# MakisChristou/fhestring

Measured on AMD Instinct MI355X. Metric: PBS/sec and ms/op for contains() on N-char FheString, higher is better.
Workload: dtype f64

## Files before the change

### __graft_entry__.py

```python
import os
import subprocess
import sys

ROOT = os.path.dirname(os.path.abspath(__file__))
if ROOT not in sys.path:
    sys.path.insert(0, ROOT)


def build():
    subprocess.check_call(["make", "-s", "-j4", "-C", os.path.join(ROOT, "fhestring_amd", "csrc")])
    subprocess.check_call(["make", "-s", "-C", os.path.join(ROOT, "oracle"), "liboracle.so"])
    subprocess.check_call(["gcc", "-std=c99", "-Wall", "-Wextra", "-pedantic", "-Werror", "-I", os.path.join(ROOT, "include"),
                           os.path.join(ROOT, "examples", "c_host.c"), "-L", os.path.join(ROOT, "fhestring_amd"),
                           "-lfhestring_hip", "-Wl,-rpath,$ORIGIN/../fhestring_amd", "-o", os.path.join(ROOT, "examples", "c_host")])
    import fhestring_amd
    fhestring_amd.lib()
    from oracle import core
    core.lib()


def smoke():
    import numpy as np
    import fhestring_amd
    from fhestring_amd.api import MyServerKey
# ... 2 lines not shown
    osk = core.ServerKey(keys)
    sk = MyServerKey.from_raw_keys(keys.bsk, keys.ksk, arith=fhestring_amd.Context.ARITH_F64_FFT)
    names = ["msg", "eq_biv", "sign"]
    luts = np.stack([radix.lut_poly(n) for n in names])
    cts = np.stack([keys.encrypt_block(m) for m in (0, 3, 9, 15, 22, 31)])
    idx = np.array([0, 1, 2, 0, 2, 1], np.uint32)
    got = sk.ctx.pbs_batch(cts, idx, luts)
    assert np.array_equal(got, osk.pbs_batch(cts, idx, luts, mode=3)), "HIP FFT PBS differs from the CPU mirror"
    sk.ctx.set_arithmetic(sk.ctx.ARITH_EXACT_NTT)
    got = sk.ctx.pbs_batch(cts, idx, luts)
    assert np.array_equal(got, osk.pbs_batch(cts, idx, luts)), "HIP PBS differs from the CPU oracle"
    osk.set_mb2(keys.bsk_mb2)
    sk.ctx.set_arithmetic(sk.ctx.ARITH_F64_FFT)
    sk.ctx.load_multibit_key(keys.bsk_mb2)
    sk.ctx.set_arithmetic(sk.ctx.ARITH_F64_FFT_MB2)
    got = sk.ctx.pbs_batch(cts, idx, luts)
    assert np.array_equal(got, osk.pbs_batch(cts, idx, luts, mode=4)), "HIP two-bit PBS differs from the CPU mirror"
    sk.ctx.set_arithmetic(sk.ctx.ARITH_EXACT_NTT)
    sk.ctx.load_multibit_key(keys.bsk_mb2)
    sk.ctx.set_arithmetic(sk.ctx.ARITH_EXACT_NTT_MB2)
    got = sk.ctx.pbs_batch(cts, idx, luts)
    assert np.array_equal(got, osk.pbs_batch(cts, idx, luts, mode=5)), "HIP exact two-bit PBS differs from the CPU oracle"
    sk.ctx.set_arithmetic(sk.ctx.ARITH_EXACT_NTT)
    sk.set_mode(1)
    s = sk.upload_string(np.stack([keys.encrypt_char(b) for b in b"zama!\0"]))
    res = sk.contains_clear(s, "ma")
    assert keys.decrypt_char(res.download()) == 1
    res = sk.contains_clear(s, "xy")
    assert keys.decrypt_char(res.download()) == 0
    sk.close()
    _smoke_rekey()
    print("smoke ok: PBS bit-exact vs oracle (exact NTT, f64 FFT, both with two key bits per product too), "
          "contains() decrypts correctly, store re-key equals the host reference and decrypts under the new key, "
          "find / rfind / len / flag counts beyond 255 decrypt correctly")


def _smoke_rekey():
    import numpy as np
    from fhestring_amd import FhsError
    from fhestring_amd.api import CompactFheString, MyClientKey, MyServerKey, rekey_host
    N = 2048
    chosen = (0x00000000, 0x00008000, 0x7FFF8000, 0x80000000, 0xFFFFFFFF, 0x00007FFF)
    a, b = MyClientKey(0x5EEDA), MyClientKey(0x5EEDB)
    sk = MyServerKey.from_client_key(a)
    sk.load_packing_key(a)
    key = a.rekey_key(b)
    sk.load_rekey_key(key)
    rng = np.random.default_rng(3)

    def words(n_blocks):
        g = (n_blocks + N - 1) // N
        mask = rng.integers(0, 1 << 32, (g, N), dtype=np.uint32)
        if g == len(chosen):
            mask[:] = np.array(chosen, np.uint32)[:, None]
        return mask, rng.integers(0, 1 << 32, n_blocks, dtype=np.uint32)
# ... 86 lines not shown
```

### bindings/fhestring_hip.rs

```rust
#![allow(non_camel_case_types, dead_code)]
use std::os::raw::{c_char, c_int, c_void};

pub const FHS_LWE_N: c_int = 742;
pub const FHS_POLY_N: c_int = 2048;
pub const FHS_BIG_CT: c_int = 2049;
pub const FHS_SMALL_CT: c_int = 743;
pub const FHS_BLOCKS_PER_CHAR: c_int = 4;
pub const FHS_CHAR_WORDS: usize = 8196;
pub const FHS_BSK_WORDS: usize = 6078464;
pub const FHS_KSK_WORDS: usize = 7608320;
pub const FHS_MAX_FIND_LENGTH: c_int = 255;
pub const FHS_MAX_REPETITIONS: c_int = 16;
pub const FHS_MAX_FIND_LENGTH_WIDE: c_int = 65535;
pub const FHS_WIDE_ABSENT: c_int = 65535;
pub const FHS_OK: c_int = 0;
pub const FHS_ERR_ARG: c_int = -1;
pub const FHS_ERR_HIP: c_int = -2;
pub const FHS_ERR_STATE: c_int = -3;
pub const FHS_ERR_LIMIT: c_int = -4;
pub const FHS_ARITH_EXACT_NTT: c_int = 0;
pub const FHS_ARITH_F64_FFT: c_int = 1;
pub const FHS_ARITH_F64_FFT_MB2: c_int = 2;
pub const FHS_ARITH_EXACT_NTT_MB2: c_int = 3;
pub const FHS_BSK_MB2_WORDS: usize = 9117696;
// ... 62 lines not shown
    pub pbs_shared: u64,
    pub pbs_extracted: u64,
}

#[link(name = "fhestring_hip")]
extern "C" {
    pub fn fhs_ctx_create(device_id: c_int, out: *mut *mut fhs_ctx) -> c_int;
    pub fn fhs_ctx_create_planner(out: *mut *mut fhs_ctx) -> c_int;
    pub fn fhs_ctx_destroy(ctx: *mut fhs_ctx);
    pub fn fhs_last_error(ctx: *const fhs_ctx) -> *const c_char;
    pub fn fhs_load_server_key(ctx: *mut fhs_ctx, bsk: *const u64, ksk: *const u64) -> c_int;
    pub fn fhs_load_multibit_key(ctx: *mut fhs_ctx, bsk_mb2: *const u64) -> c_int;
    pub fn fhs_set_arithmetic(ctx: *mut fhs_ctx, arith: c_int) -> c_int;
    pub fn fhs_get_arithmetic(ctx: *const fhs_ctx) -> c_int;
    pub fn fhs_set_fft4_max_batch(ctx: *mut fhs_ctx, max_batch: c_int) -> c_int;
    pub fn fhs_set_launch_chunk(ctx: *mut fhs_ctx, arith: c_int, n_ciphertexts: usize) -> c_int;
    pub fn fhs_fft_tables(w_re: *mut f64, w_im: *mut f64, u_re: *mut f64, u_im: *mut f64);
    pub fn fhs_fft_mono_table(mono: *mut f64);
    pub fn fhs_pbs_batch(ctx: *mut fhs_ctx, r#in: *const u64, lut_idx: *const u32, luts: *const u64, n_luts: usize, out: *mut u64, B: usize) -> c_int;
    pub fn fhs_keyswitch_modswitch_batch(ctx: *mut fhs_ctx, r#in: *const u64, ms_out: *mut u32, B: usize) -> c_int;
    pub fn fhs_pbs_batch_shifted(ctx: *mut fhs_ctx, r#in: *const u64, lut_idx: *const u32, luts: *const u64, n_luts: usize, shifts: *const u32, n_shifts: usize, out: *mut u64, B: usize) -> c_int;
    pub fn fhs_set_rotation_sharing(ctx: *mut fhs_ctx, on: c_int) -> c_int;
    pub fn fhs_debug_blind_rotate_batch(ctx: *mut fhs_ctx, ks: *const u64, lut_idx: *const u32, luts: *const u64, n_luts: usize, out: *mut u64, B: usize) -> c_int;
    pub fn fhs_pbs_batch_device(ctx: *mut fhs_ctx, d_in: *const u64, d_lut_idx: *const u32, d_luts: *const u64, d_out: *mut u64, B: usize, hip_stream: *mut c_void) -> c_int;
    pub fn fhs_kernel_timing(ctx: *mut fhs_ctx, reset: c_int, blind_rotate_ms: *mut f64, keyswitch_ms: *mut f64, n_blind_rotate: *mut u64, n_keyswitch: *mut u64, pbs_in_launches: *mut u64) -> c_int;
    pub fn fhs_kernel_timing_kind(ctx: *mut fhs_ctx, kind: c_int, avg_ms: *mut f64, launches: *mut u64, pbs_in_launches: *mut u64) -> c_int;
    pub fn fhs_trivial(ctx: *mut fhs_ctx, value: u8) -> fhs_char_t;
    pub fn fhs_upload(ctx: *mut fhs_ctx, blocks: *const u64) -> fhs_char_t;
    pub fn fhs_upload_string(ctx: *mut fhs_ctx, blocks: *const u64, n: usize, out: *mut fhs_char_t) -> c_int;
    pub fn fhs_eq(ctx: *mut fhs_ctx, a: fhs_char_t, b: fhs_char_t) -> fhs_char_t;
    pub fn fhs_ne(ctx: *mut fhs_ctx, a: fhs_char_t, b: fhs_char_t) -> fhs_char_t;
    pub fn fhs_le(ctx: *mut fhs_ctx, a: fhs_char_t, b: fhs_char_t) -> fhs_char_t;
    pub fn fhs_lt(ctx: *mut fhs_ctx, a: fhs_char_t, b: fhs_char_t) -> fhs_char_t;
    pub fn fhs_ge(ctx: *mut fhs_ctx, a: fhs_char_t, b: fhs_char_t) -> fhs_char_t;
    pub fn fhs_gt(ctx: *mut fhs_ctx, a: fhs_char_t, b: fhs_char_t) -> fhs_char_t;
    pub fn fhs_bitand(ctx: *mut fhs_ctx, a: fhs_char_t, b: fhs_char_t) -> fhs_char_t;
    pub fn fhs_bitor(ctx: *mut fhs_ctx, a: fhs_char_t, b: fhs_char_t) -> fhs_char_t;
    pub fn fhs_sub(ctx: *mut fhs_ctx, a: fhs_char_t, b: fhs_char_t) -> fhs_char_t;
    pub fn fhs_add(ctx: *mut fhs_ctx, a: fhs_char_t, b: fhs_char_t) -> fhs_char_t;
    pub fn fhs_if_then_else(ctx: *mut fhs_ctx, cond: fhs_char_t, t: fhs_char_t, f: fhs_char_t) -> fhs_char_t;
    pub fn fhs_flip(ctx: *mut fhs_ctx, a: fhs_char_t) -> fhs_char_t;
    pub fn fhs_is_whitespace(ctx: *mut fhs_ctx, a: fhs_char_t) -> fhs_char_t;
    pub fn fhs_is_uppercase(ctx: *mut fhs_ctx, a: fhs_char_t) -> fhs_char_t;
    pub fn fhs_is_lowercase(ctx: *mut fhs_ctx, a: fhs_char_t) -> fhs_char_t;
    pub fn fhs_clone(ctx: *mut fhs_ctx, a: fhs_char_t) -> fhs_char_t;
    pub fn fhs_release(ctx: *mut fhs_ctx, a: fhs_char_t) -> c_int;
// ... 161 lines not shown
```

### fhestring_amd/api.py

```python
import ctypes as C

import numpy as np

from . import cabi
from ._lib import FhsError, lib, check_single_hip_runtime

_K = dict(cabi.parse_header()["consts"])
BIG_CT = _K["FHS_BIG_CT"]
SMALL_CT = _K["FHS_SMALL_CT"]
POLY_N = _K["FHS_POLY_N"]
PACK_GROUP = _K["FHS_PACK_GROUP"]
PACK_KEY_WORDS = _K["FHS_PACK_KEY_WORDS"]
REKEY_KEY_WORDS = _K["FHS_REKEY_KEY_WORDS"]


def _ptr(a):
    return a.ctypes.data_as(C.c_void_p)


class Context:

    def __init__(self, device_id=0, planner=False):
        self._L = lib()
        if not planner:
# ... 111 lines not shown
                                          _ptr(out), B))
        return out

    def pbs_batch_shifted(self, cts, lut_idx, luts, shifts):
        cts = np.ascontiguousarray(cts, np.uint64).reshape(-1, BIG_CT)
        luts = np.ascontiguousarray(luts, np.uint64).reshape(-1, POLY_N)
        lut_idx = np.ascontiguousarray(lut_idx, np.uint32)
        B = cts.shape[0]
        shifts = np.ascontiguousarray(shifts, np.uint32).reshape(B, -1)
        out = np.zeros((B, shifts.shape[1], BIG_CT), np.uint64)
        self._check(self._L.fhs_pbs_batch_shifted(self._h, _ptr(cts), _ptr(lut_idx), _ptr(luts), luts.shape[0],
                                                  _ptr(shifts), shifts.shape[1], _ptr(out), B))
        return out

    def set_rotation_sharing(self, on=True):
        self._check(self._L.fhs_set_rotation_sharing(self._h, int(bool(on))))

    def keyswitch_modswitch_batch(self, cts):
        cts = np.ascontiguousarray(cts, np.uint64).reshape(-1, BIG_CT)
        B = cts.shape[0]
        out = np.zeros((B, SMALL_CT), np.uint32)
        self._check(self._L.fhs_keyswitch_modswitch_batch(self._h, _ptr(cts), _ptr(out), B))
        return out

    def pbs_batch_device(self, d_in, d_lut_idx, d_luts, d_out, B, stream=0):
        self._check(self._L.fhs_pbs_batch_device(self._h, C.c_void_p(d_in), C.c_void_p(d_lut_idx),
                                                 C.c_void_p(d_luts), C.c_void_p(d_out), int(B),
                                                 C.c_void_p(stream)))

    def kernel_timing(self, reset=False):
        br, ks = C.c_double(), C.c_double()
        nb, nk, units = C.c_uint64(), C.c_uint64(), C.c_uint64()
        narrow = self.kernel_timing_kind(2)
        self._check(self._L.fhs_kernel_timing(self._h, int(reset), C.byref(br), C.byref(ks), C.byref(nb),
                                              C.byref(nk), C.byref(units)))
        return {"blind_rotate_ms": br.value, "keyswitch_ms": ks.value, "n_blind_rotate": nb.value,
                "n_keyswitch": nk.value, "pbs_in_launches": units.value,
                "fft4_ms": narrow[0], "n_fft4": narrow[1], "pbs_in_fft4": narrow[2]}

    def kernel_timing_kind(self, kind):
        ms, n, u = C.c_double(), C.c_uint64(), C.c_uint64()
        self._check(self._L.fhs_kernel_timing_kind(self._h, int(kind), C.byref(ms), C.byref(n), C.byref(u)))
        return ms.value, n.value, u.value


CHAR_WORDS = _K["FHS_CHAR_WORDS"]
# ... 1122 lines not shown
```

### fhestring_amd/csrc/capi_core.cpp

```cpp
#include <algorithm>
#include <new>

#include "capi_internal.h"
#include "keyfile.h"
#include "luts.h"
#include "seeded_kernels.h"

extern "C" {

int fhs_ctx_create(int device_id, fhs_ctx **out) {
    if (!out) return FHS_ERR_ARG;
    *out = nullptr;
    fhs_ctx *c = new (std::nothrow) fhs_ctx();
    if (!c) return FHS_ERR_STATE;
    int rc = c->eng.ctx.init(device_id);
    if (rc) {
        *out = c;
        return rc;
    }
    *out = c;
    return FHS_OK;
}

int fhs_ctx_create_planner(fhs_ctx **out) {
// ... 109 lines not shown
    return e == hipSuccess ? FHS_OK : c.hip_fail(e, "device keystream");
}

int fhs_pbs_batch(fhs_ctx *ctx, const uint64_t *in, const uint32_t *lut_idx, const uint64_t *luts,
                  size_t n_luts, uint64_t *out, size_t B) {
    if (!ctx) return FHS_ERR_ARG;
    return ctx->eng.ctx.pbs_batch_host(in, lut_idx, luts, n_luts, out, B);
}

int fhs_pbs_batch_shifted(fhs_ctx *ctx, const uint64_t *in, const uint32_t *lut_idx, const uint64_t *luts, size_t n_luts,
                          const uint32_t *shifts, size_t n_shifts, uint64_t *out, size_t B) {
    if (!ctx) return FHS_ERR_ARG;
    if (ctx->eng.planner) return ctx->eng.ctx.fail(FHS_ERR_STATE, "planner context: nothing is computed");
    return ctx->eng.ctx.pbs_batch_shifted_host(in, lut_idx, luts, n_luts, shifts, n_shifts, out, B);
}

int fhs_debug_blind_rotate_batch(fhs_ctx *ctx, const uint64_t *ks, const uint32_t *lut_idx, const uint64_t *luts,
                                 size_t n_luts, uint64_t *out, size_t B) {
    if (!ctx) return FHS_ERR_ARG;
    if (ctx->eng.planner) return ctx->eng.ctx.fail(FHS_ERR_STATE, "planner context: nothing is computed");
    return ctx->eng.ctx.blind_rotate_host(ks, lut_idx, luts, n_luts, out, B);
}

int fhs_keyswitch_modswitch_batch(fhs_ctx *ctx, const uint64_t *in, uint32_t *ms_out, size_t B) {
    if (!ctx) return FHS_ERR_ARG;
    return ctx->eng.ctx.ks_ms_batch_host(in, ms_out, B);
}

int fhs_pbs_batch_device(fhs_ctx *ctx, const uint64_t *d_in, const uint32_t *d_lut_idx, const uint64_t *d_luts,
                         uint64_t *d_out, size_t B, void *hip_stream) {
    if (!ctx) return FHS_ERR_ARG;
    if (!d_in || !d_lut_idx || !d_luts || !d_out) return ctx->eng.ctx.fail(FHS_ERR_ARG, "null device pointer");
    return ctx->eng.ctx.pbs_batch_device(d_in, d_lut_idx, d_luts, d_out, B,
                                         hip_stream ? (hipStream_t)hip_stream : ctx->eng.ctx.stream);
}

int fhs_debug_capture_pbs_inputs(fhs_ctx *ctx, size_t max_rows_per_level) {
    if (!ctx) return FHS_ERR_ARG;
    if (int rc = ctx->eng.flush()) return rc;
    ctx->eng.capture_max_rows = max_rows_per_level;
    if (!max_rows_per_level) {
        ctx->eng.capture_rows.clear(); ctx->eng.capture_rows.shrink_to_fit();
        ctx->eng.capture_recs.clear();
    }
    return FHS_OK;
}
// ... 95 lines not shown
```

### fhestring_amd/csrc/context.cpp

```cpp
#include "context.h"
#include "pack_kernels.h"
#include "rekey_kernels.h"
#include "seeded_kernels.h"
#include "../../include/fhestring_hip.h"

#include <algorithm>
#include <cstdlib>
#include <utility>

namespace fhs {

namespace {
constexpr size_t KSK_BYTES = (size_t)BIG_N * KS_LEVEL * SMALL_CT * sizeof(uint64_t);
constexpr size_t BSK_BYTES = (size_t)LWE_N * 4 * POLY_N * sizeof(uint64_t);
}

#define HIP_TRY(expr, what)                                \
    do {                                                   \
        hipError_t e__ = (expr);                           \
        if (e__ != hipSuccess) return hip_fail(e__, what); \
    } while (0)

Event KernelTimer::get() {
    if (pool.empty()) return Event();
// ... 179 lines not shown
        for (int k = 0; k < 3; k++) ok = ok && ur[k] == ht.u_re[k] && ui[k] == ht.u_im[k];
        if (!ok) return fail(-3, "fft_consts.inc does not match the libm-derived twiddles (regenerate it)");
    }
    std::vector<double> flat;
    auto put = [&](const std::vector<double> &v) {
        const size_t at = flat.size();
        flat.insert(flat.end(), v.begin(), v.end());
        return at;
    };
    const size_t at_lanetab = put(ht.lanetab), at_weff = put(ht.weff), at_mono = put(ht.mono), at_r16 = put(ht.r16);
    HIP_TRY(d_fft_tables.reserve_exact(flat.size() * sizeof(double)), "hipMalloc fft tables");
    HIP_TRY(hipMemcpy(d_fft_tables.ptr, flat.data(), flat.size() * sizeof(double), hipMemcpyHostToDevice), "copy fft tables");
    const double *const tab = d_fft_tables.as<double>();
    ft.lanetab = tab + at_lanetab; ft.weff = tab + at_weff; ft.mono = tab + at_mono; ft.r16 = tab + at_r16;
    const size_t n = (size_t)LWE_N * 4 * POLY_N;
    HIP_TRY(d_bsk_fft.reserve_exact(n * sizeof(double)), "hipMalloc bsk fft");
    hipError_t e = launch_bsk_to_fft(d_bsk_std.as<uint64_t>(), d_bsk_fft.as<double>(), ft.lanetab, stream);
    if (e == hipSuccess) e = hipStreamSynchronize(stream);
    if (e != hipSuccess) d_bsk_fft.release();
    HIP_TRY(e, "bsk -> Fourier domain");
    return 0;
}

int Context::keyswitch(const uint64_t *d_in, size_t B, hipStream_t s) {
    if (dig_buf.cap < ks_digits_bytes((int)B)) {
        HIP_TRY(hipStreamSynchronize(s), "sync");
        HIP_TRY(dig_buf.reserve(ks_digits_bytes((int)B)), "hipMalloc digits");
    }
    timer.begin(1, B, s);
    hipError_t e = launch_keyswitch_mfma(d_in, d_ksk_planes.as<int8_t>(), dig_buf.as<int8_t>(), ks_buf.as<uint64_t>(), (int)B, s,
                                         wg_slots / 4);
    timer.end(s);
    if (e != hipSuccess) return hip_fail(e, "keyswitch launch");
    return 0;
}

int Context::set_arithmetic(int mode) {
    if (mode < 0 || mode >= N_ARITH) return fail(-1, "unknown arithmetic mode");
    if (is_f64_fft(mode) && key_loaded && !d_bsk_fft)
        if (int rc = build_fft_key()) return rc;
    if (mode == FHS_ARITH_F64_FFT_MB2 && key_loaded && !d_bsk_mb)
        return fail(-3, "the two-bits-per-product arithmetic needs the pair key in the Fourier domain: call "
                        "fhs_load_multibit_key while arithmetic 1 (f64 FFT) is selected, then fhs_set_arithmetic 2");
    if (mode == FHS_ARITH_EXACT_NTT_MB2 && key_loaded && !d_bsk_ntt_mb)
        return fail(-3, "the exact two-bits-per-product arithmetic needs the pair key converted to residues: call "
                        "fhs_load_multibit_key while the EXACT arithmetic (fhs_set_arithmetic 0) is selected, then "
                        "fhs_set_arithmetic 3");
    arith = mode;
    return 0;
}

int Context::load_multibit_key(const uint64_t *bsk_mb2) {
    if (!bsk_mb2) return fail(-1, "null key pointer");
    if (!key_loaded) return fail(-3, "load the server key before the pair key");
    HIP_TRY(hipSetDevice(device), "hipSetDevice");
    if (!is_f64_fft(arith)) {
// ... 208 lines not shown
                              out_buf.as<uint64_t>(), nullptr, B, stream))
        return rc;
    HIP_TRY(hipMemcpyAsync(out, out_buf.ptr, B * BIG_CT * 8, hipMemcpyDeviceToHost, stream), "D2H");
    HIP_TRY(hipStreamSynchronize(stream), "sync");
    return 0;
}

int Context::ks_ms_batch_host(const uint64_t *in, uint32_t *ms_out, size_t B) {
    if (!key_loaded) return fail(-3, "server key not loaded");
    if (!in || !ms_out) return fail(-1, "null pointer");
    if (B == 0) return 0;
    HIP_TRY(hipSetDevice(device), "hipSetDevice");
    HIP_TRY(in_buf.reserve(B * BIG_CT * 8), "hipMalloc");
    HIP_TRY(ms_buf.reserve(B * SMALL_CT * 4), "hipMalloc");
    HIP_TRY(ks_buf.reserve(B * SMALL_CT * 8), "hipMalloc");
    HIP_TRY(hipMemcpyAsync(in_buf.ptr, in, B * BIG_CT * 8, hipMemcpyHostToDevice, stream), "H2D");
    if (int rc = keyswitch(in_buf.as<uint64_t>(), B, stream)) return rc;
    HIP_TRY(launch_modswitch(ks_buf.as<uint64_t>(), ms_buf.as<uint32_t>(), (int)B, stream), "modswitch launch");
    HIP_TRY(hipMemcpyAsync(ms_out, ms_buf.ptr, B * SMALL_CT * 4, hipMemcpyDeviceToHost, stream), "D2H");
    HIP_TRY(hipStreamSynchronize(stream), "sync");
    return 0;
}

}
```

### fhestring_amd/csrc/context.h

```cpp
#pragma once
#include <hip/hip_runtime.h>

#include <cstdint>
#include <string>
#include <vector>

#include "../../include/fhestring_hip.h"
#include "dist.h"
#include "fft_tables.h"
#include "hip_owners.h"
#include "ntt_tables.h"
#include "pbs_kernels.h"

namespace fhs {

constexpr int N_ARITH = 4;
constexpr bool is_f64_fft(int arith) { return arith == FHS_ARITH_F64_FFT || arith == FHS_ARITH_F64_FFT_MB2; }

struct FftTablePtrs {
    const double *lanetab = nullptr;
    const double *weff = nullptr;
    const double *mono = nullptr;
    const double *r16 = nullptr;
};
// ... 25 lines not shown
    DevBuf d_tables;
    NttTables tw{};
    double crt_c = 0;

    int arith = FHS_ARITH_EXACT_NTT;
    DevBuf d_bsk_fft;
    DevBuf d_bsk_std;
    DevBuf d_fft_tables;
    FftTablePtrs ft;
    DevBuf d_work_counter;
    int wg_slots = 1024;
    DevBuf d_bsk_mb;
    DevBuf d_bsk_ntt_mb;
    const double *d_ntt_mono = nullptr;
    DevBuf d_pack_key_ntt;
    int load_packing_key(const uint64_t *key);
    DevBuf d_rekey_key_ntt;
    int load_rekey_key(const uint64_t *key);
    int load_multibit_key(const uint64_t *bsk_mb2);
    int fft4_max_batch = 512;
    size_t launch_chunk[N_ARITH] = {};
    int set_arithmetic(int mode);
    int keyswitch(const uint64_t *d_in, size_t B, hipStream_t s);
    int blind_rotate(const uint64_t *d_ks, const uint32_t *d_lut_idx, const uint64_t *d_luts, uint64_t *d_out,
                     uint64_t *const *d_out_ptrs, size_t B, hipStream_t s, uint64_t *const *d_body_ptrs = nullptr);

    Dist dist;
    DevBuf xchg_send, xchg_recv;

    DevBuf dig_buf;
    DevBuf ks_buf, ms_buf, in_buf, out_buf, lutidx_buf, luts_buf, tab_buf;
    DevBuf pack_ws[2], pack_tab, pack_out;
    KernelTimer timer;

    int init(int device_id);
    ~Context();
    int fail(int code, const std::string &msg) { err = msg; return code; }
    int hip_fail(hipError_t e, const char *what);

    int load_server_key(const uint64_t *bsk, const uint64_t *ksk);
    int load_compressed_server_key(const uint32_t seed[8], const uint64_t *bsk_bodies, const uint64_t *ksk_bodies);
    int install_server_key(const uint64_t *bsk, const uint64_t *d_ksk);
    int build_fft_key();
    int pbs_batch_device(const uint64_t *d_in, const uint32_t *d_lut_idx, const uint64_t *d_luts,
                         uint64_t *d_out, size_t B, hipStream_t s);
    int pbs_batch_shifted_host(const uint64_t *in, const uint32_t *lut_idx, const uint64_t *luts, size_t n_luts,
                               const uint32_t *shifts, size_t S, uint64_t *out, size_t B);
    int pbs_batch_host(const uint64_t *in, const uint32_t *lut_idx, const uint64_t *luts, size_t n_luts,
                       uint64_t *out, size_t B);
    int ks_ms_batch_host(const uint64_t *in, uint32_t *ms_out, size_t B);
    int blind_rotate_host(const uint64_t *ks, const uint32_t *lut_idx, const uint64_t *luts, size_t n_luts,
                          uint64_t *out, size_t B);
};

}
```

### fhestring_amd/csrc/engine.cpp

```cpp
#include "engine.h"
#include "../../include/fhestring_hip.h"

#include <algorithm>
#include <cstdio>
#include <cstdlib>
#include <cstring>
#include <map>

namespace fhs {

int Engine::on_key_loaded() {
    if (!d_luts_) {
        std::vector<uint64_t> host((size_t)LUT_COUNT * POLY_N);
        for (int id = 0; id < LUT_COUNT; id++) make_lut_poly(id, host.data() + (size_t)id * POLY_N);
        hipError_t e = d_luts_.reserve_exact(host.size() * 8);
        if (e != hipSuccess) return ctx.hip_fail(e, "hipMalloc luts");
        e = hipMemcpy(d_luts_.ptr, host.data(), host.size() * 8, hipMemcpyHostToDevice);
        if (e != hipSuccess) return ctx.hip_fail(e, "copy luts");
    }
    return 0;
}

Engine::~Engine() {
    if (!planner && ctx.stream) (void)hipStreamSynchronize(ctx.stream);
// ... 706 lines not shown
    const size_t stride = (cnt + capture_max_rows - 1) / capture_max_rows;
    for (size_t i = 0; i < cnt; i += stride) {
        const size_t at = capture_rows.size();
        capture_rows.resize(at + BIG_CT);
        hipError_t e = hipMemcpyAsync(capture_rows.data() + at, batch_in_.as<uint64_t>() + (batch_row + i) * BIG_CT, BIG_CT * 8,
                                      hipMemcpyDeviceToHost, ctx.stream);
        if (e == hipSuccess) e = hipStreamSynchronize(ctx.stream);
        if (e != hipSuccess) return ctx.hip_fail(e, "capture download");
        CaptureRec r = l.recs[first + i];
        r.level = level;
        capture_recs.push_back(r);
    }
    return 0;
}

int Engine::launch_rows(const GroupView &v, size_t lo, size_t cnt, uint64_t *dense_out, const TickLevel *levels,
                        size_t n_levels, size_t first_level) {
    const uint8_t *dp = tick_buf_.as<uint8_t>();
    const LinDesc *d_desc = reinterpret_cast<const LinDesc *>(dp);
    const LinTerm *d_terms = reinterpret_cast<const LinTerm *>(dp + v.off_terms);
    const uint32_t *d_lut = reinterpret_cast<const uint32_t *>(dp + v.off_lut);
    uint64_t *const *d_out = reinterpret_cast<uint64_t *const *>(dp + v.off_out);
    uint64_t *const *d_body = reinterpret_cast<uint64_t *const *>(dp + v.off_body);
    hipError_t e = launch_lincomb(d_desc + lo, d_terms, batch_in_.as<uint64_t>(), (int)cnt, ctx.stream);
    if (e != hipSuccess) return ctx.hip_fail(e, "lincomb launch");
    size_t row0 = 0;
    for (size_t j = 0; j < n_levels && capture_max_rows; j++) {
        const TickLevel &l = levels[j];
        const size_t w = l.descs.size(), a = std::max(lo, row0), b = std::min(lo + cnt, row0 + w);
        if (l.recs.size() == w && a < b)
            if (int rc = sample_capture(l, a - row0, b - a, a - lo, (uint32_t)(first_level + j))) return rc;
        row0 += w;
    }
    if (int rc = ctx.keyswitch(batch_in_.as<uint64_t>(), cnt, ctx.stream)) return rc;
    return ctx.blind_rotate(ctx.ks_buf.as<uint64_t>(), d_lut + lo, d_luts_.as<uint64_t>(), dense_out, dense_out ? nullptr : d_out + lo, cnt,
                            ctx.stream, v.n_ext && !dense_out ? d_body + lo : nullptr);
}

int Engine::scatter_rows(const uint64_t *d_all, uint64_t *const *d_out, size_t width) {
    hipError_t e = launch_scatter_blocks(d_all, d_out, (int)width, ctx.stream);
    return e == hipSuccess ? 0 : ctx.hip_fail(e, "scatter launch");
}

void Engine::trace_group(const std::vector<TickLevel> &levels, size_t width) {
    for (auto &l : levels) {
        for (size_t k = 0; k < l.descs.size(); k++) {
            const LinDesc &d = l.descs[k];
            trace_.insert(trace_.end(), {TR_ROW, (uint64_t)(uintptr_t)l.out[k], l.lut[k], d.konst_body >> DELTA_LOG, d.n_terms});
            for (uint32_t t = 0; t < d.n_terms; t++) {
                trace_.push_back((uint64_t)(uintptr_t)l.terms[d.first_term + t].src);
                trace_.push_back((uint64_t)l.terms[d.first_term + t].coef);
            }
        }
        for (const ShareRow &f : l.ext)
            trace_.insert(trace_.end(), {TR_EXT, (uint64_t)(uintptr_t)l.out[f.lead_row], (uint64_t)(uintptr_t)f.out, f.K});
    }
    trace_.push_back(TR_GROUP_END);
// ... 169 lines not shown
```

### fhestring_amd/csrc/pbs_kernels.h

```cpp
#pragma once
#include <hip/hip_runtime.h>
#include <cstddef>
#include <cstdint>

namespace fhs {

constexpr int LWE_N = 742;
constexpr int POLY_N = 2048;
constexpr int BIG_N = 2048;
constexpr int BIG_CT = 2049;
constexpr int SMALL_CT = 743;
constexpr int KS_LEVEL = 5;
constexpr int KS_BASE_LOG = 3;
constexpr int DELTA_LOG = 59;
constexpr int BSK_QUANT_BITS = 6;

constexpr uint64_t NTT_P0 = 140737488273409ull;
constexpr uint64_t NTT_P1 = 140737488252929ull;
constexpr uint64_t NTT_PSI0 = 124135596386681ull;
constexpr uint64_t NTT_PSI1 = 116052249937262ull;

struct NttTables {
    const double *fwd_uni;
    const double *fwd_lane;
// ... 71 lines not shown

size_t blind_rotate_lds_bytes();
hipError_t prepare_device_for_kernels();
hipError_t read_device_ntt_consts(double *fwd_uni , double *inv_uni , double *crt);
hipError_t launch_blind_rotate(const BlindRotateParams &p, hipStream_t s);
hipError_t launch_blind_rotate_fft(const BlindRotateFftParams &p, hipStream_t s);
hipError_t launch_blind_rotate_fft4(const BlindRotateFftParams &p, hipStream_t s);
hipError_t launch_bsk_to_fft(const uint64_t *d_bsk_std, double *d_out, const double *d_lanetab, hipStream_t s,
                             int n_polys = LWE_N * 4);
hipError_t launch_blind_rotate_mb2(const BlindRotateMb2Params &p, hipStream_t s);
hipError_t launch_blind_rotate_ntt_mb2(const BlindRotateNttMb2Params &p, hipStream_t s);
hipError_t prepare_device_for_ntt_mb2();
hipError_t prepare_device_for_fft4();
hipError_t prepare_device_for_keyswitch();
void fft_uniform_consts(double *w_re, double *w_im, double *u_re, double *u_im);
size_t ks_planes_bytes();
size_t ks_digits_bytes(int B);
hipError_t launch_ksk_to_planes(const uint64_t *d_ksk, int8_t *d_planes, hipStream_t s);
hipError_t launch_keyswitch_mfma(const uint64_t *d_in , const int8_t *d_planes, int8_t *d_dig ,
                                 uint64_t *d_ks_out , int B, hipStream_t s, int n_cus = 256);
hipError_t launch_modswitch(const uint64_t *d_ks, uint32_t *d_ms , int B, hipStream_t s);
hipError_t launch_lincomb(const LinDesc *d_desc, const LinTerm *d_terms, uint64_t *d_out ,
                          int n, hipStream_t s);
hipError_t launch_scatter_blocks(const uint64_t *d_in, uint64_t *const *d_dst, int n, hipStream_t s);
hipError_t launch_gather_rows(const uint64_t *const *d_src, uint64_t *d_out, int n, hipStream_t s);
struct ExtractDesc {
    const uint64_t *lead;
    const uint64_t *body;
    uint64_t *out;
    uint32_t K, pad;
};
hipError_t launch_extract_shift(const ExtractDesc *d_desc, int n, hipStream_t s);

}
```

### include/fhestring_hip.h

```cpp
#ifndef FHESTRING_HIP_H
#define FHESTRING_HIP_H

#include <stddef.h>
#include <stdint.h>

#ifdef __cplusplus
extern "C" {
#endif

#define FHS_LWE_N 742
#define FHS_POLY_N 2048
#define FHS_BIG_CT 2049
#define FHS_SMALL_CT 743
#define FHS_BLOCKS_PER_CHAR 4
#define FHS_CHAR_WORDS (4 * 2049)
#define FHS_BSK_WORDS ((size_t)742 * 4 * 2048)
#define FHS_KSK_WORDS ((size_t)2048 * 5 * 743)
#define FHS_MAX_FIND_LENGTH 255
#define FHS_MAX_REPETITIONS 16
#define FHS_MAX_FIND_LENGTH_WIDE 65535
#define FHS_WIDE_ABSENT 65535

#define FHS_OK 0
#define FHS_ERR_ARG (-1)
// ... 11 lines not shown
const char *fhs_last_error(const fhs_ctx *ctx);
int fhs_load_server_key(fhs_ctx *ctx, const uint64_t *bsk, const uint64_t *ksk);
#define FHS_ARITH_EXACT_NTT 0
#define FHS_ARITH_F64_FFT 1
#define FHS_ARITH_F64_FFT_MB2 2
#define FHS_ARITH_EXACT_NTT_MB2 3
#define FHS_BSK_MB2_WORDS ((size_t)371 * 3 * 4 * 2048)
int fhs_load_multibit_key(fhs_ctx *ctx, const uint64_t *bsk_mb2 );
int fhs_set_arithmetic(fhs_ctx *ctx, int arith);
int fhs_get_arithmetic(const fhs_ctx *ctx);
int fhs_set_fft4_max_batch(fhs_ctx *ctx, int max_batch);
int fhs_set_launch_chunk(fhs_ctx *ctx, int arith, size_t n_ciphertexts);
void fhs_fft_tables(double *w_re, double *w_im, double *u_re, double *u_im);
void fhs_fft_mono_table(double *mono );

int fhs_pbs_batch(fhs_ctx *ctx, const uint64_t *in, const uint32_t *lut_idx, const uint64_t *luts,
                  size_t n_luts, uint64_t *out, size_t B);
int fhs_keyswitch_modswitch_batch(fhs_ctx *ctx, const uint64_t *in, uint32_t *ms_out, size_t B);
int fhs_pbs_batch_shifted(fhs_ctx *ctx, const uint64_t *in, const uint32_t *lut_idx, const uint64_t *luts, size_t n_luts,
                          const uint32_t *shifts , size_t n_shifts, uint64_t *out, size_t B);
int fhs_set_rotation_sharing(fhs_ctx *ctx, int on);
int fhs_debug_blind_rotate_batch(fhs_ctx *ctx, const uint64_t *ks, const uint32_t *lut_idx, const uint64_t *luts,
                                 size_t n_luts, uint64_t *out, size_t B);
int fhs_pbs_batch_device(fhs_ctx *ctx, const uint64_t *d_in, const uint32_t *d_lut_idx,
                         const uint64_t *d_luts, uint64_t *d_out, size_t B, void *hip_stream);
int fhs_kernel_timing(fhs_ctx *ctx, int reset, double *blind_rotate_ms, double *keyswitch_ms,
                      uint64_t *n_blind_rotate, uint64_t *n_keyswitch, uint64_t *pbs_in_launches);
int fhs_kernel_timing_kind(fhs_ctx *ctx, int kind, double *avg_ms, uint64_t *launches, uint64_t *pbs_in_launches);

fhs_char_t fhs_trivial(fhs_ctx *ctx, uint8_t value);
fhs_char_t fhs_upload(fhs_ctx *ctx, const uint64_t *blocks );
int fhs_upload_string(fhs_ctx *ctx, const uint64_t *blocks, size_t n, fhs_char_t *out);
fhs_char_t fhs_eq(fhs_ctx *ctx, fhs_char_t a, fhs_char_t b);
fhs_char_t fhs_ne(fhs_ctx *ctx, fhs_char_t a, fhs_char_t b);
fhs_char_t fhs_le(fhs_ctx *ctx, fhs_char_t a, fhs_char_t b);
fhs_char_t fhs_lt(fhs_ctx *ctx, fhs_char_t a, fhs_char_t b);
fhs_char_t fhs_ge(fhs_ctx *ctx, fhs_char_t a, fhs_char_t b);
fhs_char_t fhs_gt(fhs_ctx *ctx, fhs_char_t a, fhs_char_t b);
fhs_char_t fhs_bitand(fhs_ctx *ctx, fhs_char_t a, fhs_char_t b);
fhs_char_t fhs_bitor(fhs_ctx *ctx, fhs_char_t a, fhs_char_t b);
fhs_char_t fhs_sub(fhs_ctx *ctx, fhs_char_t a, fhs_char_t b);
fhs_char_t fhs_add(fhs_ctx *ctx, fhs_char_t a, fhs_char_t b);
fhs_char_t fhs_if_then_else(fhs_ctx *ctx, fhs_char_t cond, fhs_char_t t, fhs_char_t f);
fhs_char_t fhs_flip(fhs_ctx *ctx, fhs_char_t a);
fhs_char_t fhs_is_whitespace(fhs_ctx *ctx, fhs_char_t a);
fhs_char_t fhs_is_uppercase(fhs_ctx *ctx, fhs_char_t a);
// ... 254 lines not shown
```

Before: 138,100.

## Fuse linear-combination pre-pass with keyswitch digit decomposition

Adds a kernel that computes the per-row linear combination of input blocks and directly decomposes it into signed keyswitch digits in the MFMA tile layout, writing only the body word to the staging buffer and zeroing the keyswitch output. This replaces the separate lincomb launch, which wrote full 2049-word ciphertexts that the keyswitch then re-read to decompose. The engine uses the fused path whenever capture sampling is off, and a debug entry point checks it against the staged path. The cost is recomputing the term sums inside a new kernel and extra coupling to the keyswitch kernels' digit layout and split logic.

Result: no change. 138,700 (median of 6 runs) (+0.4%).

```diff
diff --git a/__graft_entry__.py b/__graft_entry__.py
--- a/__graft_entry__.py
+++ b/__graft_entry__.py
@@ -48,6 +48,14 @@
     got = sk.ctx.pbs_batch(cts, idx, luts)
     assert np.array_equal(got, osk.pbs_batch(cts, idx, luts, mode=5)), "HIP exact two-bit PBS differs from the CPU oracle"
     sk.ctx.set_arithmetic(sk.ctx.ARITH_EXACT_NTT)
+    rng = np.random.default_rng(15)
+    blocks = rng.integers(0, 1 << 64, (8, 2049), dtype=np.uint64)
+    for B in (33, 129, 513):
+        n_terms = (np.arange(B) % 4).astype(np.uint32)
+        args = (n_terms, rng.integers(0, 8, int(n_terms.sum())), rng.integers(-8, 9, int(n_terms.sum())),
+                rng.integers(0, 32, B).astype(np.uint64) << np.uint64(59))
+        staged, fused = sk.ctx.lincomb_keyswitch(False, blocks, *args), sk.ctx.lincomb_keyswitch(True, blocks, *args)
+        assert all(np.array_equal(a, b) for a, b in zip(staged, fused)), "fused pre-pass differs from the staged path"
     sk.set_mode(1)
     s = sk.upload_string(np.stack([keys.encrypt_char(b) for b in b"zama!\0"]))
     res = sk.contains_clear(s, "ma")
@@ -57,6 +65,7 @@
     sk.close()
     _smoke_rekey()
     print("smoke ok: PBS bit-exact vs oracle (exact NTT, f64 FFT, both with two key bits per product too), "
+          "fused pre-pass equals lincomb + keyswitch, "
           "contains() decrypts correctly, store re-key equals the host reference and decrypts under the new key, "
           "find / rfind / len / flag counts beyond 255 decrypt correctly")
 
diff --git a/bindings/fhestring_hip.rs b/bindings/fhestring_hip.rs
--- a/bindings/fhestring_hip.rs
+++ b/bindings/fhestring_hip.rs
@@ -108,6 +108,7 @@
     pub fn fhs_pbs_batch_shifted(ctx: *mut fhs_ctx, r#in: *const u64, lut_idx: *const u32, luts: *const u64, n_luts: usize, shifts: *const u32, n_shifts: usize, out: *mut u64, B: usize) -> c_int;
     pub fn fhs_set_rotation_sharing(ctx: *mut fhs_ctx, on: c_int) -> c_int;
     pub fn fhs_debug_blind_rotate_batch(ctx: *mut fhs_ctx, ks: *const u64, lut_idx: *const u32, luts: *const u64, n_luts: usize, out: *mut u64, B: usize) -> c_int;
+    pub fn fhs_debug_lincomb_keyswitch(ctx: *mut fhs_ctx, fused: c_int, blocks: *const u64, n_blocks: usize, row_terms: *const u32, term_block: *const u32, term_coef: *const i64, row_const: *const u64, B: usize, digits: *mut u8, n_digits: *mut usize, body: *mut u64, ks_out: *mut u64) -> c_int;
     pub fn fhs_pbs_batch_device(ctx: *mut fhs_ctx, d_in: *const u64, d_lut_idx: *const u32, d_luts: *const u64, d_out: *mut u64, B: usize, hip_stream: *mut c_void) -> c_int;
     pub fn fhs_kernel_timing(ctx: *mut fhs_ctx, reset: c_int, blind_rotate_ms: *mut f64, keyswitch_ms: *mut f64, n_blind_rotate: *mut u64, n_keyswitch: *mut u64, pbs_in_launches: *mut u64) -> c_int;
     pub fn fhs_kernel_timing_kind(ctx: *mut fhs_ctx, kind: c_int, avg_ms: *mut f64, launches: *mut u64, pbs_in_launches: *mut u64) -> c_int;
diff --git a/fhestring_amd/api.py b/fhestring_amd/api.py
--- a/fhestring_amd/api.py
+++ b/fhestring_amd/api.py
@@ -157,6 +157,22 @@
         out = np.zeros((B, SMALL_CT), np.uint32)
         self._check(self._L.fhs_keyswitch_modswitch_batch(self._h, _ptr(cts), _ptr(out), B))
         return out
+
+    def lincomb_keyswitch(self, fused, blocks, row_terms, term_block, term_coef, row_const):
+        blocks = np.ascontiguousarray(blocks, np.uint64).reshape(-1, BIG_CT)
+        row_terms = np.ascontiguousarray(row_terms, np.uint32)
+        term_block = np.ascontiguousarray(term_block, np.uint32)
+        term_coef = np.ascontiguousarray(term_coef, np.int64)
+        row_const = np.ascontiguousarray(row_const, np.uint64)
+        B = row_terms.size
+        assert row_const.size == B and term_block.size == term_coef.size == int(row_terms.sum())
+        digits = np.zeros((B + 255) // 256 * 8 * 327680, np.uint8)
+        n = C.c_size_t()
+        body, ks = np.zeros(B, np.uint64), np.zeros((B, SMALL_CT), np.uint64)
+        self._check(self._L.fhs_debug_lincomb_keyswitch(self._h, int(bool(fused)), _ptr(blocks), blocks.shape[0], _ptr(row_terms),
+                                                        _ptr(term_block), _ptr(term_coef), _ptr(row_const), B, _ptr(digits),
+                                                        C.byref(n), _ptr(body), _ptr(ks)))
+        return digits[:n.value], body, ks
 
     def pbs_batch_device(self, d_in, d_lut_idx, d_luts, d_out, B, stream=0):
         self._check(self._L.fhs_pbs_batch_device(self._h, C.c_void_p(d_in), C.c_void_p(d_lut_idx),
diff --git a/fhestring_amd/csrc/capi_core.cpp b/fhestring_amd/csrc/capi_core.cpp
--- a/fhestring_amd/csrc/capi_core.cpp
+++ b/fhestring_amd/csrc/capi_core.cpp
@@ -155,6 +155,16 @@
     return ctx->eng.ctx.blind_rotate_host(ks, lut_idx, luts, n_luts, out, B);
 }
 
+int fhs_debug_lincomb_keyswitch(fhs_ctx *ctx, int fused, const uint64_t *blocks, size_t n_blocks, const uint32_t *row_terms,
+                                const uint32_t *term_block, const int64_t *term_coef, const uint64_t *row_const, size_t B,
+                                uint8_t *digits, size_t *n_digits, uint64_t *body, uint64_t *ks_out) {
+    if (!ctx) return FHS_ERR_ARG;
+    if (ctx->eng.planner) return ctx->eng.ctx.fail(FHS_ERR_STATE, "planner context: nothing is computed");
+    if (int rc = ctx->eng.flush()) return rc;
+    return ctx->eng.ctx.debug_lincomb_keyswitch(fused != 0, blocks, n_blocks, row_terms, term_block, term_coef, row_const, B,
+                                                reinterpret_cast<int8_t *>(digits), n_digits, body, ks_out);
+}
+
 int fhs_keyswitch_modswitch_batch(fhs_ctx *ctx, const uint64_t *in, uint32_t *ms_out, size_t B) {
     if (!ctx) return FHS_ERR_ARG;
     return ctx->eng.ctx.ks_ms_batch_host(in, ms_out, B);
diff --git a/fhestring_amd/csrc/context.cpp b/fhestring_amd/csrc/context.cpp
--- a/fhestring_amd/csrc/context.cpp
+++ b/fhestring_amd/csrc/context.cpp
@@ -225,16 +225,31 @@
     return 0;
 }
 
-int Context::keyswitch(const uint64_t *d_in, size_t B, hipStream_t s) {
+int Context::reserve_digits(size_t B, hipStream_t s) {
     if (dig_buf.cap < ks_digits_bytes((int)B)) {
         HIP_TRY(hipStreamSynchronize(s), "sync");
         HIP_TRY(dig_buf.reserve(ks_digits_bytes((int)B)), "hipMalloc digits");
     }
+    return 0;
+}
+
+int Context::keyswitch(const uint64_t *d_in, size_t B, hipStream_t s) {
+    if (int rc = reserve_digits(B, s)) return rc;
     timer.begin(1, B, s);
     hipError_t e = launch_keyswitch_mfma(d_in, d_ksk_planes.as<int8_t>(), dig_buf.as<int8_t>(), ks_buf.as<uint64_t>(), (int)B, s,
                                          wg_slots / 4);
     timer.end(s);
     if (e != hipSuccess) return hip_fail(e, "keyswitch launch");
+    return 0;
+}
+
+int Context::lincomb_keyswitch(const LinDesc *d_desc, const LinTerm *d_terms, uint64_t *d_stage, size_t B, hipStream_t s) {
+    if (int rc = reserve_digits(B, s)) return rc;
+    timer.begin(1, B, s);
+    hipError_t e = launch_lincomb_keyswitch(d_desc, d_terms, d_stage, d_ksk_planes.as<int8_t>(), dig_buf.as<int8_t>(),
+                                            ks_buf.as<uint64_t>(), (int)B, s, wg_slots / 4);
+    timer.end(s);
+    if (e != hipSuccess) return hip_fail(e, "fused keyswitch launch");
     return 0;
 }
 
@@ -489,4 +504,54 @@
     return 0;
 }
 
-}
+int Context::debug_lincomb_keyswitch(bool fused, const uint64_t *blocks, size_t n_blocks, const uint32_t *row_terms,
+                                     const uint32_t *term_block, const int64_t *term_coef, const uint64_t *row_const, size_t B,
+                                     int8_t *digits, size_t *n_digits, uint64_t *body, uint64_t *ks_out) {
+    if (!key_loaded) return fail(-3, "server key not loaded");
+    if (!blocks || !row_terms || !row_const || !digits || !n_digits || !body || !ks_out || B == 0 || n_blocks == 0 ||
+        B > (size_t)1 << 20)
+        return fail(-1, "bad argument");
+    std::vector<LinDesc> descs(B);
+    std::vector<LinTerm> terms;
+    HIP_TRY(hipSetDevice(device), "hipSetDevice");
+    DevBuf d_blocks, d_plan;
+    HIP_TRY(d_blocks.reserve_exact(n_blocks * BIG_CT * 8), "hipMalloc");
+    for (size_t k = 0; k < B; k++) {
+        descs[k] = LinDesc{(uint32_t)terms.size(), row_terms[k], row_const[k]};
+        for (uint32_t t = 0; t < row_terms[k]; t++) {
+            const size_t at = terms.size();
+            if (!term_block || !term_coef || term_block[at] >= n_blocks) return fail(-1, "term out of range");
+            terms.push_back(LinTerm{d_blocks.as<uint64_t>() + (size_t)term_block[at] * BIG_CT, term_coef[at]});
+        }
+    }
+    const size_t off_terms = B * sizeof(LinDesc), stage_bytes = B * BIG_CT * 8, ks_bytes = B * SMALL_CT * 8;
+    HIP_TRY(d_plan.reserve_exact(off_terms + (terms.size() + 1) * sizeof(LinTerm)), "hipMalloc");
+    HIP_TRY(in_buf.reserve(stage_bytes), "hipMalloc");
+    HIP_TRY(ks_buf.reserve(ks_bytes), "hipMalloc");
+    if (int rc = reserve_digits(B, stream)) return rc;
+    const LinDesc *d_desc = d_plan.as<LinDesc>();
+    const LinTerm *d_terms = reinterpret_cast<const LinTerm *>(d_plan.as<uint8_t>() + off_terms);
+    HIP_TRY(hipMemcpyAsync(d_blocks.ptr, blocks, n_blocks * BIG_CT * 8, hipMemcpyHostToDevice, stream), "H2D");
+    HIP_TRY(hipMemcpyAsync(d_plan.ptr, descs.data(), off_terms, hipMemcpyHostToDevice, stream), "H2D");
+    if (!terms.empty())
+        HIP_TRY(hipMemcpyAsync(d_plan.as<uint8_t>() + off_terms, terms.data(), terms.size() * sizeof(LinTerm), hipMemcpyHostToDevice,
+                               stream), "H2D");
+    HIP_TRY(hipMemsetAsync(in_buf.ptr, 0xff, stage_bytes, stream), "fill");
+    HIP_TRY(hipMemsetAsync(ks_buf.ptr, 0xff, ks_bytes, stream), "fill");
+    HIP_TRY(hipMemsetAsync(dig_buf.ptr, 0xff, ks_digits_bytes((int)B), stream), "fill");
+    if (fused) {
+        if (int rc = lincomb_keyswitch(d_desc, d_terms, in_buf.as<uint64_t>(), B, stream)) return rc;
+    } else {
+        HIP_TRY(launch_lincomb(d_desc, d_terms, in_buf.as<uint64_t>(), (int)B, stream), "lincomb launch");
+        if (int rc = keyswitch(in_buf.as<uint64_t>(), B, stream)) return rc;
+    }
+    const size_t tiles = B >= 129 ? (B + 255) / 256 * 8 : (B + 127) / 128 * 4;
+    *n_digits = tiles * (BIG_N * KS_LEVEL / 32) * 1024;
+    HIP_TRY(hipMemcpyAsync(digits, dig_buf.ptr, *n_digits, hipMemcpyDeviceToHost, stream), "D2H");
+    HIP_TRY(hipMemcpy2DAsync(body, 8, in_buf.as<uint64_t>() + BIG_N, (size_t)BIG_CT * 8, 8, B, hipMemcpyDeviceToHost, stream), "D2H");
+    HIP_TRY(hipMemcpyAsync(ks_out, ks_buf.ptr, ks_bytes, hipMemcpyDeviceToHost, stream), "D2H");
+    HIP_TRY(hipStreamSynchronize(stream), "sync");
+    return 0;
+}
+
+}
diff --git a/fhestring_amd/csrc/context.h b/fhestring_amd/csrc/context.h
--- a/fhestring_amd/csrc/context.h
+++ b/fhestring_amd/csrc/context.h
@@ -71,6 +71,8 @@
     size_t launch_chunk[N_ARITH] = {};
     int set_arithmetic(int mode);
     int keyswitch(const uint64_t *d_in, size_t B, hipStream_t s);
+    int reserve_digits(size_t B, hipStream_t s);
+    int lincomb_keyswitch(const LinDesc *d_desc, const LinTerm *d_terms, uint64_t *d_stage, size_t B, hipStream_t s);
     int blind_rotate(const uint64_t *d_ks, const uint32_t *d_lut_idx, const uint64_t *d_luts, uint64_t *d_out,
                      uint64_t *const *d_out_ptrs, size_t B, hipStream_t s, uint64_t *const *d_body_ptrs = nullptr);
 
@@ -98,6 +100,9 @@
     int pbs_batch_host(const uint64_t *in, const uint32_t *lut_idx, const uint64_t *luts, size_t n_luts,
                        uint64_t *out, size_t B);
     int ks_ms_batch_host(const uint64_t *in, uint32_t *ms_out, size_t B);
+    int debug_lincomb_keyswitch(bool fused, const uint64_t *blocks, size_t n_blocks, const uint32_t *row_terms,
+                                const uint32_t *term_block, const int64_t *term_coef, const uint64_t *row_const, size_t B,
+                                int8_t *digits, size_t *n_digits, uint64_t *body, uint64_t *ks_out);
     int blind_rotate_host(const uint64_t *ks, const uint32_t *lut_idx, const uint64_t *luts, size_t n_luts,
                           uint64_t *out, size_t B);
 };
diff --git a/fhestring_amd/csrc/engine.cpp b/fhestring_amd/csrc/engine.cpp
--- a/fhestring_amd/csrc/engine.cpp
+++ b/fhestring_amd/csrc/engine.cpp
@@ -752,17 +752,21 @@
     const uint32_t *d_lut = reinterpret_cast<const uint32_t *>(dp + v.off_lut);
     uint64_t *const *d_out = reinterpret_cast<uint64_t *const *>(dp + v.off_out);
     uint64_t *const *d_body = reinterpret_cast<uint64_t *const *>(dp + v.off_body);
-    hipError_t e = launch_lincomb(d_desc + lo, d_terms, batch_in_.as<uint64_t>(), (int)cnt, ctx.stream);
-    if (e != hipSuccess) return ctx.hip_fail(e, "lincomb launch");
-    size_t row0 = 0;
-    for (size_t j = 0; j < n_levels && capture_max_rows; j++) {
-        const TickLevel &l = levels[j];
-        const size_t w = l.descs.size(), a = std::max(lo, row0), b = std::min(lo + cnt, row0 + w);
-        if (l.recs.size() == w && a < b)
-            if (int rc = sample_capture(l, a - row0, b - a, a - lo, (uint32_t)(first_level + j))) return rc;
-        row0 += w;
-    }
-    if (int rc = ctx.keyswitch(batch_in_.as<uint64_t>(), cnt, ctx.stream)) return rc;
+    if (!capture_max_rows) {
+        if (int rc = ctx.lincomb_keyswitch(d_desc + lo, d_terms, batch_in_.as<uint64_t>(), cnt, ctx.stream)) return rc;
+    } else {
+        hipError_t e = launch_lincomb(d_desc + lo, d_terms, batch_in_.as<uint64_t>(), (int)cnt, ctx.stream);
+        if (e != hipSuccess) return ctx.hip_fail(e, "lincomb launch");
+        size_t row0 = 0;
+        for (size_t j = 0; j < n_levels; j++) {
+            const TickLevel &l = levels[j];
+            const size_t w = l.descs.size(), a = std::max(lo, row0), b = std::min(lo + cnt, row0 + w);
+            if (l.recs.size() == w && a < b)
+                if (int rc = sample_capture(l, a - row0, b - a, a - lo, (uint32_t)(first_level + j))) return rc;
+            row0 += w;
+        }
+        if (int rc = ctx.keyswitch(batch_in_.as<uint64_t>(), cnt, ctx.stream)) return rc;
+    }
     return ctx.blind_rotate(ctx.ks_buf.as<uint64_t>(), d_lut + lo, d_luts_.as<uint64_t>(), dense_out, dense_out ? nullptr : d_out + lo, cnt,
                             ctx.stream, v.n_ext && !dense_out ? d_body + lo : nullptr);
 }
diff --git a/fhestring_amd/csrc/lin_ks_kernels.hip b/fhestring_amd/csrc/lin_ks_kernels.hip
--- /dev/null
+++ b/fhestring_amd/csrc/lin_ks_kernels.hip
@@ -0,0 +1,118 @@
+#include <cstdlib>
+
+#include "pbs_kernels.h"
+
+namespace fhs {
+
+__global__ void keyswitch_mfma_kernel(const int8_t *__restrict__ dig, const int8_t *__restrict__ planes,
+                                      const uint64_t *__restrict__ in, uint64_t *__restrict__ ks_out, int B, int steps_per_split);
+__global__ void keyswitch_mfma2_kernel(const int8_t *__restrict__ dig, const int8_t *__restrict__ planes,
+                                       const uint64_t *__restrict__ in, uint64_t *__restrict__ ks_out, int B, int n_groups,
+                                       int full_blocks, int rem_tiles, int rem_slices);
+
+namespace {
+typedef int v4i __attribute__((ext_vector_type(4)));
+
+constexpr int KS_STEPS = BIG_N * KS_LEVEL / 32;
+constexpr int KS_COL_TILES = 24;
+constexpr int KS2_GROUP = 256;
+constexpr int KS2_MIN_BATCH = 129;
+constexpr int KS2_LDS_BYTES = 8 * 16 * 1024;
+
+constexpr int LK_COEFS = 64;
+constexpr int LK_CHUNKS = BIG_N / LK_COEFS;
+constexpr int LK_STEPS = LK_COEFS * KS_LEVEL / 32;
+constexpr int LK_ZCOLS = (SMALL_CT + LK_CHUNKS - 1) / LK_CHUNKS;
+static_assert(LK_COEFS * KS_LEVEL % 32 == 0 && BIG_N % LK_COEFS == 0, "whole k-steps per workgroup");
+}
+
+__device__ __forceinline__ uint64_t lin_sum(const LinDesc &d, const LinTerm *__restrict__ terms, int e) {
+    uint64_t a = 0;
+    const LinTerm *tp = terms + d.first_term;
+    for (uint32_t t = 0; t < d.n_terms; t += 4) {
+        LinTerm tm[4];
+        uint64_t x[4];
+#pragma unroll
+        for (uint32_t u = 0; u < 4; u++) tm[u] = tp[t + u < d.n_terms ? t + u : d.n_terms - 1];
+#pragma unroll
+        for (uint32_t u = 0; u < 4; u++) x[u] = tm[u].src[e];
+#pragma unroll
+        for (uint32_t u = 0; u < 4; u++) a += t + u < d.n_terms ? (uint64_t)tm[u].coef * x[u] : 0;
+    }
+    return a;
+}
+
+__global__ __launch_bounds__(256) void lincomb_digits_kernel(const LinDesc *__restrict__ desc, const LinTerm *__restrict__ terms,
+                                                             int8_t *__restrict__ dig, uint64_t *__restrict__ stage,
+                                                             uint64_t *__restrict__ ks_out, int B, int zero_from) {
+    __shared__ __attribute__((aligned(16))) int8_t frag[LK_STEPS * 1024];
+    const int tile = blockIdx.x, chunk = blockIdx.y;
+    const int lane = threadIdx.x & 63;
+    const int wave = __builtin_amdgcn_readfirstlane(threadIdx.x >> 6);
+    const int i = chunk * LK_COEFS + lane;
+    for (int q = 0; q < 8; q++) {
+        const int r = wave * 8 + q, ct = tile * 32 + r;
+        uint64_t a = 0;
+        if (ct < B) a = lin_sum(desc[ct], terms, i);
+        uint32_t v = (uint32_t)((a + (1ull << 48)) >> 49);
+#pragma unroll
+        for (int l = KS_LEVEL - 1; l >= 0; l--) {
+            int x = (int)(v & 7u);
+            v >>= 3;
+            if (x >= 4) { x -= 8; v += 1; }
+            const int k = lane * KS_LEVEL + l;
+            frag[((k >> 5) * 64 + ((k >> 4) & 1) * 32 + r) * 16 + (k & 15)] = (int8_t)x;
+        }
+    }
+    if (chunk == 0 && threadIdx.x < 32) {
+        const int ct = tile * 32 + (int)threadIdx.x;
+        if (ct < B) {
+            const LinDesc d = desc[ct];
+            stage[(size_t)ct * BIG_CT + BIG_N] = d.konst_body + lin_sum(d, terms, BIG_N);
+        }
+    }
+    for (int idx = threadIdx.x; idx < 32 * LK_ZCOLS; idx += 256) {
+        const int ct = tile * 32 + idx / LK_ZCOLS, col = chunk * LK_ZCOLS + idx % LK_ZCOLS;
+        if (ct >= zero_from && ct < B && col < SMALL_CT) ks_out[(size_t)ct * SMALL_CT + col] = 0;
+    }
+    __syncthreads();
+    v4i *dst = reinterpret_cast<v4i *>(dig + ((size_t)tile * KS_STEPS + (size_t)chunk * LK_STEPS) * 1024);
+    const v4i *src = reinterpret_cast<const v4i *>(frag);
+    for (int f = threadIdx.x; f < LK_STEPS * 64; f += 256) dst[f] = src[f];
+}
+
+hipError_t launch_lincomb_keyswitch(const LinDesc *d_desc, const LinTerm *d_terms, uint64_t *d_stage, const int8_t *d_planes,
+                                    int8_t *d_dig, uint64_t *d_ks_out, int B, hipStream_t s, int n_cus) {
+    if (B <= 0) return hipSuccess;
+    const int tiles = (B + 31) / 32;
+    static const int old_below = [] { const char *v = std::getenv("FHS_KS_OLD_BELOW"); return v ? std::atoi(v) : KS2_MIN_BATCH; }();
+    const bool wide = B >= old_below;
+    const int n_groups = (B + KS2_GROUP - 1) / KS2_GROUP, tgroups = (tiles + 3) / 4;
+    int zero_from = B, full = 0, rem = 0, slices = 1, splits = 1;
+    if (wide) {
+        const int tiles2 = KS_COL_TILES * n_groups, slots = n_cus > 0 ? n_cus : 256;
+        full = tiles2 / slots * slots;
+        rem = tiles2 - full;
+        if (rem > 0)
+            for (int c : {8, 4, 2})
+                if (rem * c <= slots) { slices = c; break; }
+        if (slices == 1) { full = tiles2; rem = 0; }
+        else zero_from = (full / 8 / 3) * KS2_GROUP;
+    } else {
+        while (splits < 16 && tgroups * KS_COL_TILES * splits < 256) splits *= 2;
+        if (splits > 1) zero_from = 0;
+    }
+    hipLaunchKernelGGL(lincomb_digits_kernel, dim3(wide ? n_groups * (KS2_GROUP / 32) : tgroups * 4, LK_CHUNKS), dim3(256), 0, s,
+                       d_desc, d_terms, d_dig, d_stage, d_ks_out, B, zero_from);
+    hipError_t e = hipGetLastError();
+    if (e != hipSuccess) return e;
+    if (wide)
+        hipLaunchKernelGGL(keyswitch_mfma2_kernel, dim3(full + rem * slices), dim3(256), KS2_LDS_BYTES, s, d_dig, d_planes,
+                           d_stage, d_ks_out, B, n_groups, full, rem > 0 ? rem : 1, slices);
+    else
+        hipLaunchKernelGGL(keyswitch_mfma_kernel, dim3(tgroups, KS_COL_TILES, splits), dim3(256), 0, s, d_dig, d_planes, d_stage,
+                           d_ks_out, B, KS_STEPS / splits);
+    return hipGetLastError();
+}
+
+}
diff --git a/fhestring_amd/csrc/pbs_kernels.h b/fhestring_amd/csrc/pbs_kernels.h
--- a/fhestring_amd/csrc/pbs_kernels.h
+++ b/fhestring_amd/csrc/pbs_kernels.h
@@ -117,6 +117,8 @@
 hipError_t launch_modswitch(const uint64_t *d_ks, uint32_t *d_ms , int B, hipStream_t s);
 hipError_t launch_lincomb(const LinDesc *d_desc, const LinTerm *d_terms, uint64_t *d_out ,
                           int n, hipStream_t s);
+hipError_t launch_lincomb_keyswitch(const LinDesc *d_desc, const LinTerm *d_terms, uint64_t *d_stage, const int8_t *d_planes,
+                                    int8_t *d_dig, uint64_t *d_ks_out , int n, hipStream_t s, int n_cus = 256);
 hipError_t launch_scatter_blocks(const uint64_t *d_in, uint64_t *const *d_dst, int n, hipStream_t s);
 hipError_t launch_gather_rows(const uint64_t *const *d_src, uint64_t *d_out, int n, hipStream_t s);
 struct ExtractDesc {
diff --git a/include/fhestring_hip.h b/include/fhestring_hip.h
--- a/include/fhestring_hip.h
+++ b/include/fhestring_hip.h
@@ -57,6 +57,10 @@
 int fhs_set_rotation_sharing(fhs_ctx *ctx, int on);
 int fhs_debug_blind_rotate_batch(fhs_ctx *ctx, const uint64_t *ks, const uint32_t *lut_idx, const uint64_t *luts,
                                  size_t n_luts, uint64_t *out, size_t B);
+int fhs_debug_lincomb_keyswitch(fhs_ctx *ctx, int fused, const uint64_t *blocks , size_t n_blocks,
+                                const uint32_t *row_terms, const uint32_t *term_block, const int64_t *term_coef,
+                                const uint64_t *row_const, size_t B, uint8_t *digits, size_t *n_digits, uint64_t *body,
+                                uint64_t *ks_out);
 int fhs_pbs_batch_device(fhs_ctx *ctx, const uint64_t *d_in, const uint32_t *d_lut_idx,
                          const uint64_t *d_luts, uint64_t *d_out, size_t B, void *hip_stream);
 int fhs_kernel_timing(fhs_ctx *ctx, int reset, double *blind_rotate_ms, double *keyswitch_ms,
```
